# immunogenomics/harmony

Measured on AMD Instinct MI355X. Metric: cells_per_sec_to_convergence, higher is better.
Workload: dtype f32

## Files before the change

### harmony_amd/csrc/hmx_api_diag.inc

```
int hmx_debug_seq_oe(const float* R, int64_t n, int32_t K, const int32_t* level, int32_t B, const int32_t* list, int64_t nlist,
                     const int32_t* chain_off, const int32_t* chain_cnt, int32_t nchains, int32_t seg_cells, int32_t passes, float* totals,
                     int64_t* mismatch, double* residual) {
  if (!R || !list || !level || !chain_off || !chain_cnt || !totals || n <= 0 || K <= 0 || B <= 0 || nchains <= 0 || seg_cells <= 0 || passes < 2) return HMX_ERR_ARG;
  if (nlist <= 0 || n > 2000000000ll || nlist > 2000000000ll || (size_t)B * 256 > 60 * 1024) return HMX_ERR_ARG;
  for (int64_t i = 0; i < nlist; i++) if (list[i] < 0 || list[i] >= n) return HMX_ERR_ARG;
  for (int64_t i = 0; i < n; i++) if (level[i] < 0 || level[i] >= B) return HMX_ERR_ARG;
  for (int c = 0; c < nchains; c++) if (chain_off[c] < 0 || chain_cnt[c] < 0 || (int64_t)chain_off[c] + chain_cnt[c] > nlist) return HMX_ERR_ARG;
  hmx_ctx* ctx = hmx_create();
  float* dR = nullptr; int* dl = nullptr; int* dlev = nullptr; int* dq = nullptr;
  auto run = [&]() -> int {
    int ndev = 0;
    if (hipGetDeviceCount(&ndev) != hipSuccess || ndev <= 0) return fail(ctx, HMX_ERR_DEVICE, "no HIP device");
    HIPCHK(hipStreamCreateWithFlags(&ctx->L.stream, hipStreamNonBlocking)); ctx->own_stream = true;
    HIPCHK(hipMalloc((void**)&dR, sizeof(float) * (size_t)n * K)); HIPCHK(hipMalloc((void**)&dl, sizeof(int) * (size_t)nlist));
    HIPCHK(hipMalloc((void**)&dlev, sizeof(int) * (size_t)n)); HIPCHK(hipMalloc((void**)&dq, sizeof(int) * (size_t)B));
    std::vector<int> ident(B); std::iota(ident.begin(), ident.end(), 0);
    CHK(h2d(ctx, dR, R, (size_t)n * K)); CHK(h2d(ctx, dl, list, (size_t)nlist)); CHK(h2d(ctx, dlev, level, (size_t)n)); CHK(h2d(ctx, dq, ident.data(), (size_t)B));
    ctx->K = K; ctx->B = B; ctx->seq_passes = passes; ctx->seq_stats = true;
    ctx->D.R = dR; ctx->D.K = K; ctx->D.B = B; ctx->D.C = 1; ctx->D.combo = dlev; ctx->D.qlev = dq;
    for (int c = 0; c < 4; c++) ctx->D.cov_end[c] = B;
    std::vector<std::pair<int, int>> ch;
    for (int c = 0; c < nchains; c++) ch.push_back({chain_off[c], chain_cnt[c]});
    CHK(seq_plan_build(ctx, ctx->plan_round, ch, seg_cells));
    CHK(seq_run_oe(ctx, ctx->plan_round, dl, nullptr, 0, nchains));
// ... 172 lines not shown
    if (!ctx->ran_setup) return -1;
    if (!out) return 64;
    std::vector<unsigned long long> h(64);
    if (d2h(ctx, h.data(), ctx->D.chain_dbg, 64)) return -1;
    (void)hipMemsetAsync(ctx->D.chain_dbg, 0, sizeof(unsigned long long) * 64, ctx->L.stream);
    return vec(h);
  }
  if (f.rfind("gputimer:", 0) == 0) {
    resolve_phases(ctx);
    const std::string nm = f.substr(9);
    if (nm == "Rcells_update") return hmx_get(ctx, "prof:update_ms", out, cap);
    auto it = ctx->gpu_timers.find(nm); return scalar(it == ctx->gpu_timers.end() ? 0.0 : it->second);
  }
  if (f.rfind("timer:", 0) == 0) { auto it = ctx->timers.find(f.substr(6)); return scalar(it == ctx->timers.end() ? 0.0 : it->second); }
  if (f == "seed_cells") return vec(ctx->seed_cells);
  if (f == "Y") return vec(ctx->Y);
  if (f == "W") return vec(ctx->W);
  if (f == "Pr_b") return vec(ctx->Pr_b);
  if (f == "theta") return vec(ctx->theta);
  if (f == "sigma") return vec(ctx->sigma);
  if (f == "lambda") return vec(ctx->lambda);
  if (f == "B_vec") return vec(ctx->B_vec);
  if (f == "objective_kmeans") return vec(ctx->obj_kmeans);
  if (f == "objective_kmeans_dist") return vec(ctx->obj_dist);
  if (f == "objective_kmeans_entropy") return vec(ctx->obj_entropy);
  if (f == "objective_kmeans_cross") return vec(ctx->obj_cross);
  if (f == "objective_harmony") return vec(ctx->obj_harmony);
  if (f == "kmeans_rounds") return vec(ctx->kmeans_rounds);
  if (ctx->query_done && (f == "Z_corr" || f == "Z_orig" || f == "R")) return hmx_get_matrix(ctx, field, out, HMX_F64, HMX_HOST, cap);
  if (!ctx->ran_setup) return -1;
// ... 151 lines not shown
```

### harmony_amd/csrc/hmx_api_kmeans.inc

```
int gather_centres(hmx_ctx* ctx, const std::vector<long long>& gcells, long long* d_gcells, double* d_rows) {
  const int K = ctx->K, d = ctx->d;
  CHK(h2d(ctx, d_gcells, gcells.data(), (size_t)K));
  l_gather_rows(ctx->L, ctx->D, d_gcells, (uint64_t)ctx->goff, d_rows); KCHK();
  CHK(allreduce(ctx, d_rows, (int64_t)K * d, 1));
  l_y_images(ctx->L, ctx->D, d_rows, 0); KCHK();
  ctx->y_on_device = true;
  return 0;
}

int kmeans_centers(hmx_ctx* ctx) {
  const int K = ctx->K, d = ctx->d;
  const Dev& D = ctx->D;
  ctx->Y.assign((size_t)d * K, 0.f);
  long long* const d_gcells = D.km_gcells; double* const d_rows = D.km_rows; unsigned* const d_excl = D.km_excl;
  std::vector<long long> gcells(K);
  const float Nm1 = (float)((uint64_t)ctx->N_global - 1);
  const bool rmode = ctx->rng_mode == 1;
  if (rmode) ensure_rrng(ctx);
  for (int i = 0; i < K; i++) gcells[i] = (long long)std::floor((rmode ? ctx->rrng.arma_randu() : hmx_u01(ctx->seed, 0, (uint64_t)i)) * Nm1);
  CHK(gather_centres(ctx, gcells, d_gcells, d_rows));
  std::vector<unsigned long long> win(K), sentinel(K, SEED_SENTINEL);
  std::set<unsigned> sup;
  if (rmode) {
    const int64_t n = ctx->N;
// ... 53 lines not shown
      CHK(h2d(ctx, D.seedmin, sentinel.data(), (size_t)K));
      CHK(seed_probe(d_excl, (int)ex.size()));
      CHK(allreduce(ctx, D.seedmin, K, 2));
      std::vector<unsigned long long> w2(K);
      CHK(d2h(ctx, w2.data(), D.seedmin, (size_t)K));
      if (w2[i] == SEED_SENTINEL) return fail(ctx, HMX_ERR_STATE, "centroid seeding ran out of distinct cells");
      g = (unsigned)(w2[i] & 0xffffffffu);
    }
    sup.insert(g);
    gcells[i] = (long long)g;
  }
  }
  ctx->seed_cells.assign(gcells.begin(), gcells.end());
  CHK(gather_centres(ctx, gcells, d_gcells, d_rows));
  const bool tile_ok = lloyd_tile_fits(D.NQ, D.NS, K, d);
  for (int it = 0; it < 10; it++) {
    if (it == 0) HIPCHK(hipMemsetAsync(D.lsum, 0, sizeof(long long) * ((size_t)K * d + K), ctx->L.stream));
    if (tile_ok) { CHK(tile_ran(ctx, TileKind::Lloyd, l_tile_static(ctx->L, D, TileKind::Lloyd))); KCHK(); }
    else { l_lloyd(ctx->L, D); KCHK(); }
    CHK(allreduce(ctx, D.lsum, (int64_t)K * d + K, 0));
    l_lloyd_finish(ctx->L, D); KCHK();
  }
  ctx->y_on_device = true;
  return 0;
}

void apply_set(Dev& D, const hmx_ctx::SortSet& s) {
  D.blk = s.blk; D.lorder = s.lorder; D.lpair = s.lpair; D.lcombo = s.lcombo; D.boff = s.boff; D.binoff = s.binoff; D.counts = s.counts; D.offs = s.offs; D.blkv = s.blkv; D.bincnt = s.bincnt;
}
int sort_group(hmx_ctx* ctx, uint64_t first) {
  const int nr = 4 - (int)(first & 3);
// ... 51 lines not shown
```

### harmony_amd/csrc/hmx_api_p2p.inc

```
int hmx_p2p_export(hmx_ctx* ctx, uint8_t* handle_out) {
  if (!ctx || !handle_out) return ctx ? fail(ctx, HMX_ERR_ARG, "null handle buffer") : HMX_ERR_ARG;
  static_assert(sizeof(hipIpcMemHandle_t) == HMX_P2P_HANDLE_BYTES, "HIP IPC handle size");
  if (ctx->device < 0) { int cur = 0; (void)hipGetDevice(&cur); ctx->device = cur; }
  HIPCHK(hipSetDevice(ctx->device));
  if (!ctx->p2p_self) {
    const char* m = getenv("HMX_P2P_MEM");
    const unsigned flags = (m && std::string(m) == "uncached") ? hipDeviceMallocUncached : hipDeviceMallocFinegrained;
    void* p = nullptr;
    HIPCHK(hipExtMallocWithFlags(&p, P2P_INBOX_GRANULES * sizeof(unsigned long long), flags));
    HIPCHK(hipMemset(p, 0, P2P_INBOX_GRANULES * sizeof(unsigned long long)));
    HIPCHK(hipDeviceSynchronize());
    ctx->p2p_self = (unsigned long long*)p;
  }
  hipIpcMemHandle_t h;
  HIPCHK(hipIpcGetMemHandle(&h, ctx->p2p_self));
  std::memcpy(handle_out, &h, sizeof(h));
  return 0;
}
int hmx_p2p_connect(hmx_ctx* ctx, int32_t rank, int32_t world, const uint8_t* handles) {
  if (!ctx || !handles) return ctx ? fail(ctx, HMX_ERR_ARG, "null handle table") : HMX_ERR_ARG;
  if (world < 2 || world > 8 || rank < 0 || rank >= world) return fail(ctx, HMX_ERR_ARG, "the peer-to-peer chain takes 2..8 ranks");
  if (!ctx->p2p_self) return fail(ctx, HMX_ERR_STATE, "hmx_p2p_export first");
  HIPCHK(hipSetDevice(ctx->device));
  for (int g = 0; g < world; g++) {
// ... 124 lines not shown
  else if (f == "seq_passes") { if (v < 2 || v > 64) return fail(ctx, HMX_ERR_ARG, "seq_passes: 2..64"); ctx->seq_passes = (int)v; if (ctx->seq_max_passes < (int)v) ctx->seq_max_passes = (int)v; }
  else if (f == "seq_warm_passes") { if (v < 1 || v > 64) return fail(ctx, HMX_ERR_ARG, "seq_warm_passes: 1..64"); ctx->seq_warm_passes = (int)v; }
  else if (f == "seq_stats") ctx->seq_stats = v != 0;
  else if (f == "seq_fused") { ctx->obj_fused = (int)(v & 1); ctx->ridge_kl = (int)((v >> 2) & 1); ctx->obj_dist_cache = (int)((v >> 3) & 1); }
  else if (f == "seq_tol_ppb") { if (v < 0 || v > 100000000) return fail(ctx, HMX_ERR_ARG, "seq_tol_ppb: 0 .. 1e8 (parts per billion)"); ctx->seq_tol = 1e-9 * (double)v; }
  else if (f == "seq_strict") { ctx->seq_strict = v != 0; if (v && ctx->seq_max_passes < 64) ctx->seq_max_passes = 64; }
  else if (f == "seq_max_passes") { if (v < 2 || v > 256) return fail(ctx, HMX_ERR_ARG, "seq_max_passes: 2..256"); ctx->seq_max_passes = (int)v; }
  else if (f == "project_slab_bytes") { if (v < 0) return fail(ctx, HMX_ERR_ARG, "project_slab_bytes: 0 (the default) or a positive byte count"); ctx->project_slab_bytes = v; }
  else if (f == "ranksum_list_bytes") { if (v < 0) return fail(ctx, HMX_ERR_ARG, "ranksum_list_bytes: 0 (the default) or a positive byte count"); ctx->ranksum_list_bytes = v; }
  else if (f == "device") ctx->device = (int)v;
  else if (f == "profile") { ctx->profile = (int)(v < 0 ? 0 : v > 2 ? 2 : v); ctx->prof_update_ms = 0; ctx->prof_update_launches = 0; ctx->prof_update_cells = 0; ctx->prof_update_steps = 0; ctx->ev_used = 0;
                             ctx->ph_used = 0; ctx->gpu_timers.clear(); }
  else if (f == "grid") { if (ctx->ran_setup) return fail(ctx, HMX_ERR_STATE, "grid must be set before setup"); ctx->L.grid = (int)v; }
  else if (f == "comm_force") ctx->comm_force = v != 0;
  else if (f == "upd_wps") { if (ctx->ran_setup) return fail(ctx, HMX_ERR_STATE, "upd_wps must be set before setup"); ctx->tun_wps = (int)v; }
  else if (f == "upd_debug") { if (ctx->ran_setup) ctx->D.upd_debug = (int)v; }
  else if (f == "upd_tpw") { ctx->tun_tpw = (int)v; if (ctx->ran_setup) ctx->D.upd_tpw = (int)(v < 1 ? 1 : v); }
  else return fail(ctx, HMX_ERR_ARG, "unknown or read-only field: " + f);
  return 0;
}
```

### harmony_amd/csrc/hmx_api_seam.inc

```
struct XferPool {
  std::vector<std::thread> th;
  const char* src = nullptr; char* dst = nullptr; size_t bytes = 0;
  std::atomic<size_t> next{0};
  std::atomic<int> gen{0}, running{0};
  std::atomic<bool> stop{false};
  static constexpr size_t CHUNK = 1 << 20;
  void work() {
    for (;;) {
      const size_t off = next.fetch_add(CHUNK);
      if (off >= bytes) break;
      memcpy(dst + off, src + off, std::min(CHUNK, bytes - off));
    }
  }
  void loop() {
    int seen = 0;
    for (;;) {
      int g;
      while ((g = gen.load(std::memory_order_acquire)) == seen) {
        if (stop.load(std::memory_order_relaxed)) return;
        __builtin_ia32_pause();
      }
      seen = g;
      work();
      running.fetch_sub(1, std::memory_order_release);
// ... 79 lines not shown
  int64_t N = 0;
  int d = 0, K = 0, B = 0, C = 0, Q = 0;
  std::vector<int> B_vec, cov_bounds;
  std::vector<float> sigma, theta, lambda, Pr_b, sizes;
  bool lambda_estimation = false;
  float alpha = 0.2f, block_size = 0.05f, eps_k = 1e-3f, eps_h = 1e-2f, cutoff = 1e-5f;
  int max_iter_kmeans = 4, window_size = 3, verbose = 0;
  uint64_t seed = 0, round_counter = 0;
  int nb = 20; uint64_t cells_per_block = 1;
  std::vector<float> Y;
  std::vector<float> W; int W_rows = 0;
  std::vector<float> obj_kmeans, obj_dist, obj_entropy, obj_cross, obj_harmony;
  std::vector<int> kmeans_rounds;
  std::vector<int> qlev, perm;
  std::vector<long long> seed_cells;
  std::deque<std::vector<int64_t>> injected;
  int64_t subset_clusters = 0, skipped_clusters = 0;
  double* h_obj = nullptr; int obj_cap = 0, obj_pending = 0; hipEvent_t obj_event = nullptr; bool obj_harmony_pending = false;
  int rng_mode = 0; hmx::RRng rrng; bool rrng_seeded = false;
  bool solve_on_device = true, y_on_device = false, solve_pending = false;
  double* sv_cov = nullptr; double* sv_rhs = nullptr; float* sv_Wall = nullptr; int* sv_mrows = nullptr; int* sv_flags = nullptr;
  float* sv_lambda = nullptr; int* sv_cov_bounds = nullptr;
  int ridge_arith = 0, oe_arith = 0, obj_arith = 0, solve_arith = 0;
  int stale_dist = 0; float* Zc_head = nullptr; float* Yt_head = nullptr; bool head_is_stale = false;
  struct SeqPlan { SeqSeg* d_segs = nullptr; SeqChain* d_chains = nullptr; size_t cap_segs = 0, cap_chains = 0; int nsegs = 0, nchains = 0;
                   std::vector<int> seg0;    int seg_cells = 0; std::vector<int> cells;    };
  SeqPlan plan_head, plan_ridge, plan_round, plan_pair;
  int* pairlist = nullptr; int* pair_idx = nullptr; int npairs = 0;
  float* rg_tot = nullptr; float* rp_tot = nullptr; float* rp_start = nullptr; bool rp_warm = false;
  float* sq_start = nullptr; float* sq_end = nullptr; size_t sq_cap = 0;
// ... 331 lines not shown
```

### harmony_amd/csrc/hmx_api_setup.inc

```
static int phi_codes(hmx_ctx* ctx, int64_t N, const int32_t* phi_i, const int32_t* phi_p, const double* phi_x, int32_t B, int32_t C,
                     std::vector<int>& codes) {
  codes.assign((size_t)C * N, 0);
  for (int64_t i = 0; i < N; i++) {
    if (phi_p[i + 1] - phi_p[i] != C) return fail(ctx, HMX_ERR_PHI, "Phi column does not hold exactly one level per covariate");
    for (int c = 0; c < C; c++) {
      const int b = phi_i[phi_p[i] + c];
      if (b < 0 || b >= B || b >= ctx->cov_bounds[c] || (c > 0 && b < ctx->cov_bounds[c - 1]))
        return fail(ctx, HMX_ERR_PHI, "Phi rows are not grouped by covariate");
      if (phi_x && phi_x[phi_p[i] + c] != 1.0) return fail(ctx, HMX_ERR_PHI, "Phi must be a 0/1 design");
      codes[(size_t)c * N + i] = b;
    }
  }
  return 0;
}
static int combo_keys(hmx_ctx* ctx, int64_t N, int32_t C, const std::vector<int>& codes, std::vector<int>& key, std::vector<long long>& present) {
  double dense = 1; for (int c = 0; c < C; c++) dense *= ctx->B_vec[c];
  if (dense > 16777216.0) return fail(ctx, HMX_ERR_LIMIT, "product of covariate level counts exceeds 2^24");
  present.assign((size_t)dense, 0);
  key.assign((size_t)N, 0);
  for (int64_t i = 0; i < N; i++) {
    int64_t kk = 0, mul = 1;
    for (int c = 0; c < C; c++) { kk += mul * (codes[(size_t)c * N + i] - (c ? ctx->cov_bounds[c - 1] : 0)); mul *= ctx->B_vec[c]; }
    key[i] = (int)kk; present[(size_t)kk]++;
  }
// ... 233 lines not shown
    const size_t bins = (size_t)P.nkeys * Q, parts = (size_t)shuffle_parts((uint64_t)ctx->N_global, D.nb, ctx->cells_per_block);
    for (int i = 0; i < 4; i++) { CHK(dalloc(ctx, &ctx->posr[i], (size_t)ctx->N_global)); CHK(dalloc(ctx, &ctx->shuf_partcnt[i], bins * parts));
      CHK(dalloc(ctx, &ctx->shuf_binacc[i], bins)); HIPCHK(hipMemsetAsync(ctx->shuf_binacc[i], 0, sizeof(int) * bins, st)); }
  }
  CHK(dalloc(ctx, &D.items, G.items.size())); CHK(dalloc(ctx, &D.aitems, G.aitems.size())); CHK(dalloc(ctx, &D.titems, G.titems.size())); CHK(dalloc(ctx, &D.qstart, (size_t)Q + 1));
  CHK(dalloc(ctx, &D.Sq, (size_t)Q * d * K)); CHK(dalloc(ctx, &D.nq, (size_t)Q * K)); CHK(dalloc(ctx, &D.S0, (size_t)K * d)); CHK(dalloc(ctx, &D.n0, (size_t)K));
  CHK(dalloc(ctx, &D.Wq, (size_t)Q * K * d)); CHK(dalloc(ctx, &D.Wimg, D.moe_mfma ? (size_t)Q * D.wNQ * D.wNS * 256 : 1));
  CHK(dalloc(ctx, &D.solve_err, (size_t)1)); HIPCHK(hipMemsetAsync(D.solve_err, 0, sizeof(int), st));
  if (ctx->solve_on_device) {
    CHK(dalloc(ctx, &ctx->sv_cov, (size_t)K * M * M)); CHK(dalloc(ctx, &ctx->sv_rhs, (size_t)K * d * M)); CHK(dalloc(ctx, &ctx->sv_Wall, (size_t)K * d * M));
    CHK(dalloc(ctx, &ctx->sv_mrows, (size_t)K)); CHK(dalloc(ctx, &ctx->sv_flags, (size_t)K)); CHK(dalloc(ctx, &ctx->sv_lambda, M)); CHK(dalloc(ctx, &ctx->sv_cov_bounds, (size_t)C));
    HIPCHK(hipMemsetAsync(ctx->sv_flags, 0, sizeof(int) * (size_t)K, st)); HIPCHK(hipMemsetAsync(ctx->sv_mrows, 0, sizeof(int) * (size_t)K, st));
  }
  CHK(dalloc(ctx, &D.km_gcells, (size_t)K)); CHK(dalloc(ctx, &D.km_rows, (size_t)K * d)); CHK(dalloc(ctx, &D.km_excl, (size_t)K));
  CHK(dalloc(ctx, &D.seedmin, (size_t)K)); CHK(dalloc(ctx, &D.lsum, (size_t)K * d + K)); D.lcnt = reinterpret_cast<unsigned long long*>(D.lsum + (size_t)K * d); CHK(dalloc(ctx, &D.ynorm, (size_t)K));
  ctx->Zc_head = nullptr; ctx->Yt_head = nullptr; ctx->head_is_stale = false;
  if (ctx->stale_dist) { CHK(dalloc(ctx, &ctx->Zc_head, N * D.zs)); CHK(dalloc(ctx, &ctx->Yt_head, (size_t)d * K)); }
  HIPCHK(hipMemsetAsync(D.R, 0, sizeof(float) * N * K, st)); HIPCHK(hipMemsetAsync(D.Zo, 0, sizeof(float) * N * D.zs, st));
  HIPCHK(hipMemsetAsync(D.Zc, 0, sizeof(float) * N * D.zs, st)); HIPCHK(hipMemsetAsync(D.Wq, 0, sizeof(float) * (size_t)Q * K * d, st));
  return 0;
}

static int upload_stats_slots(hmx_ctx* ctx, const Design& G) {
  Dev& D = ctx->D;
  const int nt = D.ntitems, Q = D.Q;
  std::vector<int> slot0((size_t)D.st_nwg), qptr((size_t)Q + 1, 0), qslots;
  std::vector<std::vector<int>> byq((size_t)Q);
  int nslots = 0;
  for (int w = 0; w < D.st_nwg; w++) {
    slot0[w] = nslots;
// ... 106 lines not shown
```

### harmony_amd/csrc/hmx_internal.h

```cpp
#pragma once
#include <hip/hip_runtime.h>
#include <stdint.h>
#include "hmx_group_plan.h"

namespace hmx {

constexpr int WAVE = 64;
constexpr int TPB = 256;
constexpr int ITEM_CELLS = 256;
constexpr int APPLY_CELLS = 1024;
constexpr int SORT_CHUNK = 512;
constexpr float FX_SCALE = 536870912.0f;
constexpr double FX_INV = 1.0 / 536870912.0;

struct Item { int q; int start; int cnt; };

struct Dev {
  int n;
  int d, K, B, C, Q;
  int B0;
  int cov_end[4];
  int dot_bf;
  int KP;
  int zs;
// ... 99 lines not shown
  int* st_qptr; int* st_qslots;
  double* S0;
  double* n0;
  int* qstart;
  float* sizes;
  float* Wq;
  float* Wimg;
  int wNQ, wNT4, wtail, wNS;
  int moe_mfma;
  long long* km_gcells; double* km_rows; unsigned* km_excl;
  unsigned long long* seedmin;
  long long* lsum;
  int usig;
  unsigned long long* lcnt;
  float* ynorm;
};

struct SolveArgs {
  double* cov; double* rhs;
  float* Wall; int* mrows; int* flags;
  int* err;
  const float* lambda;
  const int* cov_bounds;
  float alpha, cutoff; int use_s0;
  const float* Of; const float* Ef;
  const float* ref_tot; const float* pair_tot; const int* pair_idx;
  int solve_f32;
  size_t lds_b_bytes;
  size_t lds_body_bytes;
  size_t lds_mask_off;
// ... 271 lines not shown
```

### harmony_amd/csrc/hmx_k_correct.inc

```
#if !HMX_TILE_BF
__global__ __launch_bounds__(TPB) void k_objective_tables(Dev D) {
  __shared__ double red[TPB];
  const int K = D.K, B = D.B;
  double cross = 0.0;
  for (int k = threadIdx.x; k < K; k += blockDim.x) {
    long long rs = 0;
    for (int b = 0; b < B; b++) {
      if (b < D.B0) rs += D.O_fx[(size_t)b * K + k];
    }
    const double rsd = (double)rs * FX_INV;
    double ck = 0.0;
    for (int b = 0; b < B; b++) {
      const double od = (double)D.O_fx[(size_t)b * K + k] * FX_INV;
      const float o = (float)od, e = (float)(rsd * (double)D.Pr_b[b]);
      const float m = D.theta[b] * logf((o + e + 1.0f) / ((2.0f * e) + 1.0f));
      ck += od * (double)m;
    }
    cross += ck * (double)D.sigma[k];
  }
  red[threadIdx.x] = cross;
  __syncthreads();
  for (int off = TPB / 2; off > 0; off >>= 1) {
    if (threadIdx.x < off) red[threadIdx.x] += red[threadIdx.x + off];
    __syncthreads();
// ... 1001 lines not shown
          const int kb = (int)(best & 0xffffffffu);
#pragma unroll
          for (int t = 0; t < DPL; t++) {
            const int jj = 64 * t + lane;
            if (jj < d) atomicAdd((unsigned long long*)&D.lsum[(size_t)kb * d + jj], (unsigned long long)__float2ll_rn(z[c][t] * 1073741824.0f));
          }
          if (lane == 0) atomicAdd(&D.lcnt[kb], 1ull);
        }
      }
    }
  }
}

__global__ __launch_bounds__(64) void k_lloyd_finish(Dev D) {
  const int k = blockIdx.x, lane = threadIdx.x, d = D.d, K = D.K;
  const unsigned long long cnt = D.lcnt[k];
  float s2 = 0.0f;
  for (int j = lane; j < d; j += 64) {
    float y = D.Ycur[(size_t)k * d + j];
    if (cnt > 0) y = (float)(((double)D.lsum[(size_t)k * d + j] * (1.0 / 1073741824.0)) / (double)cnt);
    D.lsum[(size_t)k * d + j] = 0;
    D.Ycur[(size_t)k * d + j] = y;
    D.Yt[(size_t)j * K + k] = y;
    D.Yimg[yimg_index(D, j, k)] = y;
    bfimg_store_all(D, j, k, y);
    s2 += y * y;
  }
  __shared__ float ys[128];
  for (int j = lane; j < d; j += 64) ys[j] = D.Ycur[(size_t)k * d + j];
  __syncthreads();
  if (lane == 0) { float s = 0.0f; for (int j = 0; j < d; j++) s += ys[j] * ys[j]; D.ynorm[k] = s; D.lcnt[k] = 0ull; }
  (void)s2;
}

__global__ __launch_bounds__(64) void k_y_images(Dev D, const double* __restrict__ rows, int normalise) {
  const int k = blockIdx.x, lane = threadIdx.x, d = D.d, K = D.K;
  __shared__ float ys[128];
  __shared__ float nrm_;
  for (int j = lane; j < d; j += 64) ys[j] = rows ? (float)rows[(size_t)k * d + j] : D.Ycur[(size_t)k * d + j];
  __syncthreads();
  if (lane == 0) {
    float s = 0.0f;
    for (int j = 0; j < d; j++) s = __fadd_rn(s, __fmul_rn(ys[j], ys[j]));
    float nn = sqrtf(s);
    if (nn == 0.0f) nn = 1.0f;
    nrm_ = normalise ? nn : 1.0f;
// ... 18 lines not shown
```

### harmony_amd/csrc/hmx_k_tile.inc

```

__device__ __forceinline__ float dpp_f(float v, const int ctrl_id) {
  const int x = __float_as_int(v);
  int r;
  switch (ctrl_id) {
    case 0: r = __builtin_amdgcn_update_dpp(0, x, 0xB1, 0xF, 0xF, true); break;
    case 1: r = __builtin_amdgcn_update_dpp(0, x, 0x4E, 0xF, 0xF, true); break;
    case 2: r = __builtin_amdgcn_update_dpp(0, x, 0x141, 0xF, 0xF, true); break;
    default: r = __builtin_amdgcn_update_dpp(0, x, 0x140, 0xF, 0xF, true); break;
  }
  return __int_as_float(r);
}
__device__ __forceinline__ float rowsum16(float v) {
  v += dpp_f(v, 0);
  v += dpp_f(v, 1);
  v += dpp_f(v, 2);
  v += dpp_f(v, 3);
  return v;
}

template <int NF>
__global__ __launch_bounds__(TPB) void k_normalize4(const float* Zsrc, float* Z, int n, int nq) {
  const int lane = threadIdx.x & 63, c = lane & 15, g = lane >> 4;
  const int wave = (blockIdx.x * blockDim.x + threadIdx.x) >> 6, nw = (gridDim.x * blockDim.x) >> 6;
  const f32x4 zero4 = {0.f, 0.f, 0.f, 0.f};
// ... 535 lines not shown
  }
  unsigned long long best[MODE == 3 ? NCT : 1], sk[MODE == 3 ? NCT : 1];
  if constexpr (MODE == 3) {
#pragma unroll
    for (int ct = 0; ct < NCT; ct++) {
      best[ct] = ~0ull;
      sk[ct] = splitmix64(D.seed_key ^ ((uint64_t)(1 + kcol(NCT, ct, c)) * 0xD1342543DE82EF95ull));
    }
  }
  auto CE = [&](int ct) -> float { return ce[USIG ? 0 : ct]; };
  auto CL = [&](int ct) -> float { return cl[USIG ? 0 : ct]; };
  double od = 0.0, oe = 0.0;
  int curq = -1;
  auto tile_q = [&](const int2 cq) -> int { return __builtin_amdgcn_readfirstlane(cq.y); };
  const RowRegs* erows = nullptr;
  const int QMASK = D.qmask;
  auto flush_run = [&]() __attribute__((always_inline)) {
    long long* t2 = nullptr;
    if (UPD && D.Sold_next) t2 = D.Sold_next + (size_t)((curq >> 19) & 63) * D.B * KS + kb;
    if (MODE == 1 && D.head_gather && D.Sold_head) t2 = D.Sold_head + (size_t)((curq >> 25) & 63) * D.B * KS;
#ifdef HMX_TRACE
    if (D.upd_debug & 16) t2 = nullptr;
    if (D.upd_debug & 8) {
#pragma unroll
      for (int ct = 0; ct < NCT; ct++) oacc[ct] = 0ull;
      return;
    }
#endif
    flush_tile_fx<NCT>(snew, t2, qlevT, curq & QMASK, C, K, KS, c, g, oacc);
  };
// ... 195 lines not shown
    }
  };
  auto store_rows = [&](const int cellA, const f32x4 (&acc)[NCT]) __attribute__((always_inline)) {
#ifdef HMX_TRACE
    if (D.upd_debug & 4) return;
#endif
    if (NOSTORE || !D.r_store) return;
#pragma unroll
    for (int i = 0; i < 4; i++) {
      const int cell = __shfl(cellA, 4 * g + i, 64);
      put_row(D.R + (size_t)(cell >= 0 ? cell : D.n) * KS + kb, acc, i);
    }
  };
  auto epilogue = [&](const int cellA, const int q0, f32x4 (&acc)[NCT]) __attribute__((always_inline)) {
    if constexpr (MODE == 2) {
      float bs[4]; int bk[4];
#pragma unroll
      for (int reg = 0; reg < 4; reg++) {
        bs[reg] = INFINITY; bk[reg] = 0x7fffffff;
#pragma unroll
        for (int ct = 0; ct < NCT; ct++) {
          const float sc = (ct < first_partial_ct(NCT) || kcol(NCT, ct, c) < K) ? fmaf(acc[ct][reg], -2.0f, ce[ct]) : INFINITY;
          const bool lt = sc < bs[reg];
          bs[reg] = lt ? sc : bs[reg];
          bk[reg] = lt ? kcol(NCT, ct, c) : bk[reg];
        }
      }
      float m[4];
#pragma unroll
      for (int reg = 0; reg < 4; reg++) m[reg] = bs[reg];
#pragma unroll
      for (int st = 0; st < 4; st++) {
        float t[4];
#pragma unroll
        for (int reg = 0; reg < 4; reg++) t[reg] = (st == 0) ? dpp_f(m[reg], 0) : (st == 1) ? dpp_f(m[reg], 1) : (st == 2) ? dpp_f(m[reg], 2) : dpp_f(m[reg], 3);
#pragma unroll
        for (int reg = 0; reg < 4; reg++) m[reg] = fminf(m[reg], t[reg]);
      }
      int kb[4];
#pragma unroll
      for (int reg = 0; reg < 4; reg++) kb[reg] = (bs[reg] == m[reg]) ? bk[reg] : 0x7fffffff;
#pragma unroll
      for (int st = 0; st < 4; st++) {
        int t[4];
#pragma unroll
        for (int reg = 0; reg < 4; reg++) {
          const float kf = __int_as_float(kb[reg]);
          t[reg] = __float_as_int((st == 0) ? dpp_f(kf, 0) : (st == 1) ? dpp_f(kf, 1) : (st == 2) ? dpp_f(kf, 2) : dpp_f(kf, 3));
        }
#pragma unroll
        for (int reg = 0; reg < 4; reg++) kb[reg] = min(kb[reg], t[reg]);
      }
      const int dd = D.d;
      const float* const Zcp = D.Zc;
      if (erows) {
        int t4[4];
#pragma unroll
        for (int reg = 0; reg < 4; reg++) t4[reg] = __shfl(kb[reg], 16 * (c >> 2), 64);
        const int kc = ((c & 3) == 0) ? t4[0] : ((c & 3) == 1) ? t4[1] : ((c & 3) == 2) ? t4[2] : t4[3];
        if (cellA >= 0) {
          long long* row = ltab + (size_t)kc * dd;
          if constexpr (BF) {
#pragma unroll
            for (int t = 0; t < 4; t++) {
#pragma unroll
              for (int e = 0; e < 4; e++) {
                const int jj = 32 * (t >> 1) + 8 * g + 4 * (t & 1) + e;
                if (t < 2 * D.NS2 && jj < dd) atomicAdd((unsigned long long*)&row[jj], (unsigned long long)(long long)__float2int_rn(erows->v[t][e] * 1073741824.0f));
              }
            }
            if (g == 0) atomicAdd((unsigned long long*)&ltab[K * dd + kc], 1ull);
            return;
          }
#pragma unroll
          for (int t = 0; t < 4; t++) {
            if (t < D.NT4) {
#pragma unroll
              for (int e = 0; e < 4; e++) {
                const int jj = 16 * t + 4 * g + e;
                if (jj < dd) atomicAdd((unsigned long long*)&row[jj], (unsigned long long)(long long)__float2int_rn(erows->v[t][e] * 1073741824.0f));
              }
            }
          }
#pragma unroll
          for (int u = 0; u < 3; u++) {
            const int jj = 16 * D.NT4 + 4 * u + g;
            if (u < D.tail && jj < dd) atomicAdd((unsigned long long*)&row[jj], (unsigned long long)(long long)__float2int_rn(erows->t[u] * 1073741824.0f));
          }
          if (g == 0) atomicAdd((unsigned long long*)&ltab[K * dd + kc], 1ull);
        }
        return;
      }
      int cellr[4];
#pragma unroll
      for (int reg = 0; reg < 4; reg++) cellr[reg] = __shfl(cellA, 4 * g + reg, 64);
      for (int j0 = 0; j0 < dd; j0 += 64) {
        float z[4][4];
#pragma unroll
        for (int reg = 0; reg < 4; reg++) {
          const float* zr = Zcp + (size_t)max(cellr[reg], 0) * zs;
#pragma unroll
          for (int u = 0; u < 4; u++) z[reg][u] = zr[min(j0 + 16 * u + c, dd - 1)];
        }
#pragma unroll
        for (int reg = 0; reg < 4; reg++) {
#pragma unroll
          for (int u = 0; u < 4; u++) {
            const int jj = j0 + 16 * u + c;
            if (cellr[reg] >= 0 && jj < dd) {
              const unsigned long long v = (unsigned long long)(long long)__float2int_rn(z[reg][u] * 1073741824.0f);
              atomicAdd((unsigned long long*)&ltab[kb[reg] * dd + jj], v);
            }
          }
        }
      }
#pragma unroll
      for (int reg = 0; reg < 4; reg++)
        if (c == 0 && cellr[reg] >= 0) atomicAdd((unsigned long long*)&ltab[K * dd + kb[reg]], 1ull);
    } else if constexpr (MODE == 3) {
      int gc[4]; bool ok[4];
#pragma unroll
      for (int reg = 0; reg < 4; reg++) {
        const int cell = __shfl(cellA, 4 * g + reg, 64);
        ok[reg] = cell >= 0;
        gc[reg] = D.perm[max(cell, 0)];
      }
#pragma unroll
      for (int reg = 0; reg < 4; reg++) {
        const uint64_t gg = D.seed_goff + (uint64_t)gc[reg];
        bool skip = !ok[reg];
        for (int x = 0; x < D.seed_nexcl; x++) skip |= ((uint64_t)D.seed_excl[x] == gg);
#pragma unroll
        for (int ct = 0; ct < NCT; ct++) {
// ... 577 lines not shown
      atomicAdd(&D.chain_dbg[4], wq); atomicAdd(&D.chain_dbg[5], wg); atomicAdd(&D.chain_dbg[6], ww); atomicAdd(&D.chain_dbg[7], wd); atomicAdd(&D.chain_dbg[8], wm);
      atomicAdd(&D.chain_dbg[9], w1); atomicAdd(&D.chain_dbg[10], w2); atomicAdd(&D.chain_dbg[11], w3);
    }
    if ((blockIdx.x == 0 || blockIdx.x == 100) && lane == 0 && D.chain_dbg) {
      const int o = (blockIdx.x == 0 ? 16 : 32) + (tid >> 6);
      atomicAdd(&D.chain_dbg[o], wv_busy); atomicAdd(&D.chain_dbg[o + 8], wv_tiles);
    }
    if (blockIdx.x == 0 && (tid == 256 || tid == 320) && D.chain_dbg) {
      unsigned long long* const o = D.chain_dbg + (tid == 256 ? 48 : 56);
      atomicAdd(&o[0], wq); atomicAdd(&o[1], wg); atomicAdd(&o[2], ww); atomicAdd(&o[3], wd); atomicAdd(&o[4], wm); atomicAdd(&o[5], w1); atomicAdd(&o[6], w2); atomicAdd(&o[7], w3);
    }
    return;
    }
  }
  if (pre && (!DUAL || MODE == 2)) {
    for (int tile = ts; tile < te; tile += tstep) {
      const int2 cellA = cellN;
      const RowRegs rowsA = rowsN;
      cellN = cellNN;
      cellNN = tile_cell(tile + 2 * tstep);
      ld_rows(next_rows(cellN, cellA), rowsN);
      f32x4 acc[NCT];
      dots_regs(rowsA, cellA.x >= 0, acc);
      if constexpr (MODE == 2) erows = &rowsA;
      epilogue(cellA.x, tile_q(cellA), acc);
    }
  } else if (pre) {
    auto norm_rows = [&](RowRegs& r, const int cell) __attribute__((always_inline)) {
      if constexpr (BF) {
        const f32x4 zero4 = {0.f, 0.f, 0.f, 0.f};
        float ss = 0.0f;
#pragma unroll
        for (int t = 0; t < 4; t++) {
          r.v[t] = (rowmask >> t) & 1 ? r.v[t] : zero4;
          ss += r.v[t][0] * r.v[t][0] + r.v[t][1] * r.v[t][1] + r.v[t][2] * r.v[t][2] + r.v[t][3] * r.v[t][3];
        }
        ss += __shfl_xor(ss, 16, 64);
// ... 79 lines not shown
      epilogue(cellC.x, tile_q(cellC), accC);
      stamp(5);
    }
  } else {
    for (int tile = ts; tile < te; tile += tstep) {
      const int2 cellA = cellN;
      cellN = cellNN;
      cellNN = tile_cell(tile + 2 * tstep);
      f32x4 acc[NCT];
      dots_stream(D.Zc + (size_t)(cellA.x >= 0 ? cellA.x : 0) * zs, cellA.x >= 0, acc);
      epilogue(cellA.x, tile_q(cellA), acc);
    }
  }
  if constexpr (MODE == 2) {
    __syncthreads();
    for (int i = threadIdx.x; i < K * D.d; i += blockDim.x)
      if (ltab[i]) atomicAdd((unsigned long long*)&D.lsum[i], (unsigned long long)ltab[i]);
    for (int i = threadIdx.x; i < K; i += blockDim.x)
      if (ltab[K * D.d + i]) atomicAdd(&D.lcnt[i], (unsigned long long)ltab[K * D.d + i]);
  } else if constexpr (MODE == 3) {
#pragma unroll
    for (int ct = 0; ct < NCT; ct++) {
      unsigned long long v = best[ct];
      unsigned long long o = shfl_xor_u64(v, 16); v = o < v ? o : v;
      o = shfl_xor_u64(v, 32); v = o < v ? o : v;
      if (g == 0 && kcol(NCT, ct, c) < K && v != ~0ull) atomicMin(&D.seedmin[kcol(NCT, ct, c)], v);
    }
  } else {
    if (ts >= te) return;
    if (curq >= 0) flush_run();
// ... 15 lines not shown
```

### include/harmony_mi355x_lab.h

```cpp
#ifndef HARMONY_MI355X_LAB_H
#define HARMONY_MI355X_LAB_H

#include "harmony_mi355x.h"

#ifdef __cplusplus
extern "C" {
#endif



void hmx_r_runif(uint32_t seed, int32_t n, double* out);
void hmx_r_shuffle(uint32_t seed, int64_t N, int64_t* out);
void hmx_mt19937_by_array(const uint32_t* key, int32_t len, int32_t n, uint32_t* out);
float hmx_u01(uint64_t seed, uint64_t stream, uint64_t idx);
int32_t hmx_cluster_of_column(int32_t nct, int32_t ct, int32_t c);

int hmx_debug_seq_oe(const float* R, int64_t n, int32_t K, const int32_t* level, int32_t B, const int32_t* list, int64_t nlist,
                     const int32_t* chain_off, const int32_t* chain_cnt, int32_t nchains, int32_t seg_cells, int32_t passes, float* totals,
                     int64_t* mismatch, double* residual);
int hmx_debug_seq_arr(const float* T, int64_t n, int32_t narr, int32_t seg_terms, int32_t passes, float* total, int64_t* mismatch, double* residual);


#ifdef __cplusplus
}
#endif
#endif
```

Baseline: 76.51 million.

## Make Lloyd k-means iterations incremental by accumulating only moved cells' deltas

Stores each cell's previous cluster assignment and keeps running per-cluster sums and counts across Lloyd iterations. After the first iteration, only cells whose assignment changed contribute, adding their row to the new cluster and subtracting it from the old one, which cuts the atomic accumulation traffic. The trade-off is an extra per-cell assignment buffer read and write, and doubled atomics for the cells that do move. Counters for moved cells and debug flags are also added.

```diff
diff --git a/harmony_amd/csrc/hmx_api_diag.inc b/harmony_amd/csrc/hmx_api_diag.inc
--- a/harmony_amd/csrc/hmx_api_diag.inc
+++ b/harmony_amd/csrc/hmx_api_diag.inc
@@ -210,6 +210,16 @@
   }
   if (f.rfind("timer:", 0) == 0) { auto it = ctx->timers.find(f.substr(6)); return scalar(it == ctx->timers.end() ? 0.0 : it->second); }
   if (f == "seed_cells") return vec(ctx->seed_cells);
+  if (f == "lloyd_incremental") return scalar((double)ctx->lloyd_incremental);
+  if (f == "lloyd:on_tile") return scalar(ctx->lloyd_on_tile ? 1.0 : 0.0);
+  if (f == "lloyd:tile_pairs") return scalar(0.0);
+  if (f == "lloyd:moved") {
+    if (!ctx->ran_setup) return -1;
+    if (!out) return 10;
+    std::vector<unsigned long long> h(10);
+    if (d2h(ctx, h.data(), ctx->D.lmoved, 10)) return -1;
+    return vec(h);
+  }
   if (f == "Y") return vec(ctx->Y);
   if (f == "W") return vec(ctx->W);
   if (f == "Pr_b") return vec(ctx->Pr_b);
diff --git a/harmony_amd/csrc/hmx_api_kmeans.inc b/harmony_amd/csrc/hmx_api_kmeans.inc
--- a/harmony_amd/csrc/hmx_api_kmeans.inc
+++ b/harmony_amd/csrc/hmx_api_kmeans.inc
@@ -91,7 +91,11 @@
   ctx->seed_cells.assign(gcells.begin(), gcells.end());
   CHK(gather_centres(ctx, gcells, d_gcells, d_rows));
   const bool tile_ok = lloyd_tile_fits(D.NQ, D.NS, K, d);
+  const bool by_moves = tile_ok && ctx->lloyd_incremental;
+  ctx->lloyd_on_tile = tile_ok;
+  HIPCHK(hipMemsetAsync(D.lmoved, 0, sizeof(unsigned long long) * 16, ctx->L.stream));
   for (int it = 0; it < 10; it++) {
+    ctx->D.lloyd_first = it == 0; ctx->D.lloyd_delta = (by_moves && it > 0) ? 1 : 0; ctx->D.lloyd_it = it;
     if (it == 0) HIPCHK(hipMemsetAsync(D.lsum, 0, sizeof(long long) * ((size_t)K * d + K), ctx->L.stream));
     if (tile_ok) { CHK(tile_ran(ctx, TileKind::Lloyd, l_tile_static(ctx->L, D, TileKind::Lloyd))); KCHK(); }
     else { l_lloyd(ctx->L, D); KCHK(); }
diff --git a/harmony_amd/csrc/hmx_api_p2p.inc b/harmony_amd/csrc/hmx_api_p2p.inc
--- a/harmony_amd/csrc/hmx_api_p2p.inc
+++ b/harmony_amd/csrc/hmx_api_p2p.inc
@@ -162,6 +162,7 @@
   else if (f == "grid") { if (ctx->ran_setup) return fail(ctx, HMX_ERR_STATE, "grid must be set before setup"); ctx->L.grid = (int)v; }
   else if (f == "comm_force") ctx->comm_force = v != 0;
   else if (f == "upd_wps") { if (ctx->ran_setup) return fail(ctx, HMX_ERR_STATE, "upd_wps must be set before setup"); ctx->tun_wps = (int)v; }
+  else if (f == "lloyd_incremental") ctx->lloyd_incremental = v != 0;
   else if (f == "upd_debug") { if (ctx->ran_setup) ctx->D.upd_debug = (int)v; }
   else if (f == "upd_tpw") { ctx->tun_tpw = (int)v; if (ctx->ran_setup) ctx->D.upd_tpw = (int)(v < 1 ? 1 : v); }
   else return fail(ctx, HMX_ERR_ARG, "unknown or read-only field: " + f);
diff --git a/harmony_amd/csrc/hmx_api_seam.inc b/harmony_amd/csrc/hmx_api_seam.inc
--- a/harmony_amd/csrc/hmx_api_seam.inc
+++ b/harmony_amd/csrc/hmx_api_seam.inc
@@ -117,6 +117,8 @@
   std::vector<int> kmeans_rounds;
   std::vector<int> qlev, perm;
   std::vector<long long> seed_cells;
+  int lloyd_incremental = 1;
+  bool lloyd_on_tile = false;
   std::deque<std::vector<int64_t>> injected;
   int64_t subset_clusters = 0, skipped_clusters = 0;
   double* h_obj = nullptr; int obj_cap = 0, obj_pending = 0; hipEvent_t obj_event = nullptr; bool obj_harmony_pending = false;
diff --git a/harmony_amd/csrc/hmx_api_setup.inc b/harmony_amd/csrc/hmx_api_setup.inc
--- a/harmony_amd/csrc/hmx_api_setup.inc
+++ b/harmony_amd/csrc/hmx_api_setup.inc
@@ -271,6 +271,8 @@
   }
   CHK(dalloc(ctx, &D.km_gcells, (size_t)K)); CHK(dalloc(ctx, &D.km_rows, (size_t)K * d)); CHK(dalloc(ctx, &D.km_excl, (size_t)K));
   CHK(dalloc(ctx, &D.seedmin, (size_t)K)); CHK(dalloc(ctx, &D.lsum, (size_t)K * d + K)); D.lcnt = reinterpret_cast<unsigned long long*>(D.lsum + (size_t)K * d); CHK(dalloc(ctx, &D.ynorm, (size_t)K));
+  CHK(dalloc(ctx, &D.lassign, N)); CHK(dalloc(ctx, &D.ltot, (size_t)K * d + K)); CHK(dalloc(ctx, &D.lmoved, (size_t)16));
+  HIPCHK(hipMemsetAsync(D.lmoved, 0, sizeof(unsigned long long) * 16, st));
   ctx->Zc_head = nullptr; ctx->Yt_head = nullptr; ctx->head_is_stale = false;
   if (ctx->stale_dist) { CHK(dalloc(ctx, &ctx->Zc_head, N * D.zs)); CHK(dalloc(ctx, &ctx->Yt_head, (size_t)d * K)); }
   HIPCHK(hipMemsetAsync(D.R, 0, sizeof(float) * N * K, st)); HIPCHK(hipMemsetAsync(D.Zo, 0, sizeof(float) * N * D.zs, st));
diff --git a/harmony_amd/csrc/hmx_internal.h b/harmony_amd/csrc/hmx_internal.h
--- a/harmony_amd/csrc/hmx_internal.h
+++ b/harmony_amd/csrc/hmx_internal.h
@@ -137,6 +137,10 @@
   int usig;
   unsigned long long* lcnt;
   float* ynorm;
+  unsigned short* lassign;
+  long long* ltot;
+  unsigned long long* lmoved;
+  int lloyd_first, lloyd_delta, lloyd_it;
 };
 
 struct SolveArgs {
diff --git a/harmony_amd/csrc/hmx_k_correct.inc b/harmony_amd/csrc/hmx_k_correct.inc
--- a/harmony_amd/csrc/hmx_k_correct.inc
+++ b/harmony_amd/csrc/hmx_k_correct.inc
@@ -1039,11 +1039,14 @@
 
 __global__ __launch_bounds__(64) void k_lloyd_finish(Dev D) {
   const int k = blockIdx.x, lane = threadIdx.x, d = D.d, K = D.K;
-  const unsigned long long cnt = D.lcnt[k];
+  long long* const tcnt = D.ltot + (size_t)K * d;
+  const unsigned long long cnt = (unsigned long long)((D.lloyd_delta ? tcnt[k] : 0ll) + (long long)D.lcnt[k]);
   float s2 = 0.0f;
   for (int j = lane; j < d; j += 64) {
     float y = D.Ycur[(size_t)k * d + j];
-    if (cnt > 0) y = (float)(((double)D.lsum[(size_t)k * d + j] * (1.0 / 1073741824.0)) / (double)cnt);
+    const long long tot = (D.lloyd_delta ? D.ltot[(size_t)k * d + j] : 0ll) + D.lsum[(size_t)k * d + j];
+    D.ltot[(size_t)k * d + j] = tot;
+    if (cnt > 0) y = (float)(((double)tot * (1.0 / 1073741824.0)) / (double)cnt);
     D.lsum[(size_t)k * d + j] = 0;
     D.Ycur[(size_t)k * d + j] = y;
     D.Yt[(size_t)j * K + k] = y;
@@ -1054,7 +1057,7 @@
   __shared__ float ys[128];
   for (int j = lane; j < d; j += 64) ys[j] = D.Ycur[(size_t)k * d + j];
   __syncthreads();
-  if (lane == 0) { float s = 0.0f; for (int j = 0; j < d; j++) s += ys[j] * ys[j]; D.ynorm[k] = s; D.lcnt[k] = 0ull; }
+  if (lane == 0) { float s = 0.0f; for (int j = 0; j < d; j++) s += ys[j] * ys[j]; D.ynorm[k] = s; tcnt[k] = (long long)cnt; D.lcnt[k] = 0ull; }
   (void)s2;
 }
 
diff --git a/harmony_amd/csrc/hmx_k_tile.inc b/harmony_amd/csrc/hmx_k_tile.inc
--- a/harmony_amd/csrc/hmx_k_tile.inc
+++ b/harmony_amd/csrc/hmx_k_tile.inc
@@ -573,6 +573,12 @@
   int curq = -1;
   auto tile_q = [&](const int2 cq) -> int { return __builtin_amdgcn_readfirstlane(cq.y); };
   const RowRegs* erows = nullptr;
+  int nmoved = 0;
+  int aold = 0, aoldN = 0;
+  auto ld_assign = [&](const int cell) -> int {
+    if constexpr (MODE == 2) return (cell >= 0 && !D.lloyd_first) ? (int)D.lassign[cell] : 0;
+    else return 0;
+  };
   const int QMASK = D.qmask;
   auto flush_run = [&]() __attribute__((always_inline)) {
     long long* t2 = nullptr;
@@ -798,6 +804,9 @@
   };
   auto epilogue = [&](const int cellA, const int q0, f32x4 (&acc)[NCT]) __attribute__((always_inline)) {
     if constexpr (MODE == 2) {
+      const bool first = D.lloyd_first != 0, delta = D.lloyd_delta != 0;
+      unsigned short* const asg = D.lassign;
+      const int kold_c = (cellA < 0 || first) ? -1 : erows ? aold : (int)asg[cellA];
       float bs[4]; int bk[4];
 #pragma unroll
       for (int reg = 0; reg < 4; reg++) {
@@ -824,6 +833,12 @@
       int kb[4];
 #pragma unroll
       for (int reg = 0; reg < 4; reg++) kb[reg] = (bs[reg] == m[reg]) ? bk[reg] : 0x7fffffff;
+#ifdef HMX_TRACE
+      const bool no_argmin = (D.upd_debug & 64) != 0;
+#else
+      constexpr bool no_argmin = false;
+#endif
+      if (!no_argmin) {
 #pragma unroll
       for (int st = 0; st < 4; st++) {
         int t[4];
@@ -835,49 +850,93 @@
 #pragma unroll
         for (int reg = 0; reg < 4; reg++) kb[reg] = min(kb[reg], t[reg]);
       }
+      } else {
+#pragma unroll
+        for (int reg = 0; reg < 4; reg++) kb[reg] = min(bk[reg], K - 1);
+      }
+#ifdef HMX_TRACE
+      if (D.upd_debug & 32) return;
+#endif
       const int dd = D.d;
       const float* const Zcp = D.Zc;
+      auto fx = [](const float z, const bool neg) -> unsigned long long {
+        const int v = __float2int_rn(z * 1073741824.0f);
+        return (unsigned long long)(long long)(neg ? -v : v);
+      };
       if (erows) {
         int t4[4];
 #pragma unroll
         for (int reg = 0; reg < 4; reg++) t4[reg] = __shfl(kb[reg], 16 * (c >> 2), 64);
         const int kc = ((c & 3) == 0) ? t4[0] : ((c & 3) == 1) ? t4[1] : ((c & 3) == 2) ? t4[2] : t4[3];
-        if (cellA >= 0) {
-          long long* row = ltab + (size_t)kc * dd;
+        const bool valid = cellA >= 0;
+        const int kold = kold_c;
+        const bool mv = valid && kc != kold;
+        nmoved += __popcll(__ballot(mv && g == 0));
+        if (mv && g == 0) asg[cellA] = (unsigned short)kc;
+        const bool add = delta ? mv : valid;
+        auto add_row = [&](const int k, const bool neg) __attribute__((always_inline)) {
+          long long* row = ltab + (size_t)k * dd;
           if constexpr (BF) {
 #pragma unroll
             for (int t = 0; t < 4; t++) {
 #pragma unroll
               for (int e = 0; e < 4; e++) {
                 const int jj = 32 * (t >> 1) + 8 * g + 4 * (t & 1) + e;
-                if (t < 2 * D.NS2 && jj < dd) atomicAdd((unsigned long long*)&row[jj], (unsigned long long)(long long)__float2int_rn(erows->v[t][e] * 1073741824.0f));
+                if (t < 2 * D.NS2 && jj < dd) atomicAdd((unsigned long long*)&row[jj], fx(erows->v[t][e], neg));
               }
             }
-            if (g == 0) atomicAdd((unsigned long long*)&ltab[K * dd + kc], 1ull);
-            return;
-          }
-#pragma unroll
-          for (int t = 0; t < 4; t++) {
-            if (t < D.NT4) {
-#pragma unroll
-              for (int e = 0; e < 4; e++) {
-                const int jj = 16 * t + 4 * g + e;
-                if (jj < dd) atomicAdd((unsigned long long*)&row[jj], (unsigned long long)(long long)__float2int_rn(erows->v[t][e] * 1073741824.0f));
+          } else {
+#pragma unroll
+            for (int t = 0; t < 4; t++) {
+              if (t < D.NT4) {
+#pragma unroll
+                for (int e = 0; e < 4; e++) {
+                  const int jj = 16 * t + 4 * g + e;
+                  if (jj < dd) atomicAdd((unsigned long long*)&row[jj], fx(erows->v[t][e], neg));
+                }
               }
             }
-          }
-#pragma unroll
-          for (int u = 0; u < 3; u++) {
-            const int jj = 16 * D.NT4 + 4 * u + g;
-            if (u < D.tail && jj < dd) atomicAdd((unsigned long long*)&row[jj], (unsigned long long)(long long)__float2int_rn(erows->t[u] * 1073741824.0f));
-          }
-          if (g == 0) atomicAdd((unsigned long long*)&ltab[K * dd + kc], 1ull);
+#pragma unroll
+            for (int u = 0; u < 3; u++) {
+              const int jj = 16 * D.NT4 + 4 * u + g;
+              if (u < D.tail && jj < dd) atomicAdd((unsigned long long*)&row[jj], fx(erows->t[u], neg));
+            }
+          }
+          if (g == 0) atomicAdd((unsigned long long*)&ltab[K * dd + k], neg ? ~0ull : 1ull);
+        };
+        if (!delta) {
+          if (add) add_row(kc, false);
+          return;
+        }
+        unsigned long long todo = __ballot(mv && g == 0);
+        while (todo) {
+          const int sl = __builtin_ctzll(todo);
+          todo &= todo - 1;
+          const int cm = __builtin_amdgcn_readlane(cellA, sl), kn = min(__builtin_amdgcn_readlane(kc, sl), K - 1), ko = min(max(__builtin_amdgcn_readlane(kold, sl), 0), K - 1);
+          const float* zr = Zcp + (size_t)cm * zs;
+          for (int jj = lane; jj < dd; jj += 64) {
+            const float z = zr[jj];
+            atomicAdd((unsigned long long*)&ltab[(size_t)kn * dd + jj], fx(z, false));
+            atomicAdd((unsigned long long*)&ltab[(size_t)ko * dd + jj], fx(z, true));
+          }
+          if (lane < 2) atomicAdd((unsigned long long*)&ltab[K * dd + (lane ? ko : kn)], lane ? ~0ull : 1ull);
         }
         return;
       }
-      int cellr[4];
+      int cellr[4], kold[4]; bool mv[4];
 #pragma unroll
       for (int reg = 0; reg < 4; reg++) cellr[reg] = __shfl(cellA, 4 * g + reg, 64);
+      bool any = false;
+#pragma unroll
+      for (int reg = 0; reg < 4; reg++) {
+        kold[reg] = __shfl(kold_c, 4 * g + reg, 64);
+        mv[reg] = cellr[reg] >= 0 && kb[reg] != kold[reg];
+        kold[reg] = min(max(kold[reg], 0), K - 1);
+        nmoved += __popcll(__ballot(mv[reg] && c == 0));
+        if (mv[reg] && c == 0) asg[cellr[reg]] = (unsigned short)kb[reg];
+        any |= delta ? mv[reg] : cellr[reg] >= 0;
+      }
+      if (__ballot(any) == 0ull) return;
       for (int j0 = 0; j0 < dd; j0 += 64) {
         float z[4][4];
 #pragma unroll
@@ -891,16 +950,19 @@
 #pragma unroll
           for (int u = 0; u < 4; u++) {
             const int jj = j0 + 16 * u + c;
-            if (cellr[reg] >= 0 && jj < dd) {
-              const unsigned long long v = (unsigned long long)(long long)__float2int_rn(z[reg][u] * 1073741824.0f);
-              atomicAdd((unsigned long long*)&ltab[kb[reg] * dd + jj], v);
+            if ((delta ? mv[reg] : cellr[reg] >= 0) && jj < dd) {
+              atomicAdd((unsigned long long*)&ltab[kb[reg] * dd + jj], fx(z[reg][u], false));
+              if (delta) atomicAdd((unsigned long long*)&ltab[kold[reg] * dd + jj], fx(z[reg][u], true));
             }
           }
         }
       }
 #pragma unroll
       for (int reg = 0; reg < 4; reg++)
-        if (c == 0 && cellr[reg] >= 0) atomicAdd((unsigned long long*)&ltab[K * dd + kb[reg]], 1ull);
+        if (c == 0 && (delta ? mv[reg] : cellr[reg] >= 0)) {
+          atomicAdd((unsigned long long*)&ltab[K * dd + kb[reg]], 1ull);
+          if (delta) atomicAdd((unsigned long long*)&ltab[K * dd + kold[reg]], ~0ull);
+        }
     } else if constexpr (MODE == 3) {
       int gc[4]; bool ok[4];
 #pragma unroll
@@ -1508,13 +1570,21 @@
     }
   }
   if (pre && (!DUAL || MODE == 2)) {
+    if (ts < te) aoldN = ld_assign(cellN.x);
     for (int tile = ts; tile < te; tile += tstep) {
       const int2 cellA = cellN;
       const RowRegs rowsA = rowsN;
       cellN = cellNN;
       cellNN = tile_cell(tile + 2 * tstep);
       ld_rows(next_rows(cellN, cellA), rowsN);
+      aold = aoldN; aoldN = ld_assign(cellN.x);
       f32x4 acc[NCT];
+#ifdef HMX_TRACE
+      if (MODE == 2 && (D.upd_debug & 128)) {
+#pragma unroll
+        for (int ct = 0; ct < NCT; ct++) acc[ct] = rowsA.v[ct & 3];
+      } else
+#endif
       dots_regs(rowsA, cellA.x >= 0, acc);
       if constexpr (MODE == 2) erows = &rowsA;
       epilogue(cellA.x, tile_q(cellA), acc);
@@ -1624,6 +1694,14 @@
   }
   if constexpr (MODE == 2) {
     __syncthreads();
+    unsigned* const wmoved = reinterpret_cast<unsigned*>(lds4);
+    if (lane == 0) wmoved[threadIdx.x >> 6] = (unsigned)nmoved;
+    __syncthreads();
+    if (threadIdx.x == 0) {
+      unsigned long long m = 0;
+      for (int w = 0; w < (int)(blockDim.x >> 6); w++) m += wmoved[w];
+      if (m) atomicAdd(&D.lmoved[D.lloyd_it], m);
+    }
     for (int i = threadIdx.x; i < K * D.d; i += blockDim.x)
       if (ltab[i]) atomicAdd((unsigned long long*)&D.lsum[i], (unsigned long long)ltab[i]);
     for (int i = threadIdx.x; i < K; i += blockDim.x)
diff --git a/include/harmony_mi355x_lab.h b/include/harmony_mi355x_lab.h
--- a/include/harmony_mi355x_lab.h
+++ b/include/harmony_mi355x_lab.h
@@ -21,6 +21,7 @@
 int hmx_debug_seq_arr(const float* T, int64_t n, int32_t narr, int32_t seg_terms, int32_t passes, float* total, int64_t* mismatch, double* residual);
 
 
+
 #ifdef __cplusplus
 }
 #endif
```

Result: no change. 76.89 million, median of 5 (+0.5%).
